# darrenjkt/SEE-VCN

Hardware: AMD Instinct MI355X
Metric: scenes/sec (VCN+voxel+spconv fwd+bwd) (higher is better)
Workload: dtype f32; 1 GPU; VCN_VC fwd on 64 objects x 1024 pts -> kNN surface select (k=30) -> largest DBSCAN cluster (eps 0.4) -> unique + replace (<0.1 m) into 16 KITTI-shaped 64-beam scenes (21.0k pts in range each) -> DynMeanVFE -> VoxelBackBone8x + HeightCompression fwd+bwd + SGD (BASELINE configs[1]+[2]); scenes_per_gpu=16, objects_per_gpu=64, points_per_object=1024, geometry=KITTI [0,-40,-3,70.4,40,1] @ [0.05,0.05,0.1] -> sparse [41,1600,1408], parallelism=dp1, input_side=side stream, one batch ahead (every step = 1 front + 1 compute)

## Files before the change

### include/seevcn_hip.h

```cpp
#ifndef SEEVCN_HIP_H
#define SEEVCN_HIP_H

#include <stddef.h>
#include <stdint.h>

#ifdef __cplusplus
extern "C" {
#endif

#define SV_OK 0
#define SV_ERR_ARG 1
#define SV_ERR_HIP 2

#define SV_ABI_VERSION 1

int sv_abi_version(void);
const char* sv_last_error(void);
int sv_measure_build(void);

size_t sv_index_persistent_bytes(int64_t ncells);
size_t sv_index_scratch_bytes(int64_t ncells);

size_t sv_voxelize_dynamic_scratch_bytes(int64_t num_points, int64_t ncells, int64_t capacity);
int sv_voxelize_dynamic(const float* points, int64_t num_points, int point_stride, int num_features,
// ... 32 lines not shown
int sv_gemm_tn(const float* A, int64_t lda, const float* B, int64_t ldb, float* C, int64_t ldc, int64_t M, int N, int K, void* scratch, void* stream);
size_t sv_gemm_strided_scratch_bytes(int rows, int cols, int64_t contraction);
int sv_gemm_strided(const float* A, int64_t stride_a_row, int64_t stride_a_c, const float* B, int64_t stride_b_c, int64_t stride_b_col, float* C, int64_t ldc,
                    int rows, int cols, int64_t contraction, void* scratch, void* stream);
size_t sv_column_sums_scratch_bytes(int64_t M, int N);
int sv_column_sums(const float* A, int64_t lda, int64_t M, int N, float* out, void* scratch, void* stream);
int sv_segment_max(const float* x, int64_t ldx, int groups, int rows_per_group, int channels, float* out, int32_t* arg, void* stream);
int sv_segment_max_backward(const float* dout, const int32_t* arg, int groups, int rows_per_group, int channels, float* dx, int64_t ldx, void* stream);
int sv_segment_sum(const float* x, int64_t ldx, int groups, int rows_per_group, int channels, float* out, void* stream);
int sv_act_backward(const float* dy, const float* y, int64_t n, int act, float slope, float* dz, void* stream);

int sv_vcn_vc_prep(const float* input, int batch, int n, float* fview, float* centred, float* state, void* stream);
int sv_vcn_vc_pose(const float* fview, int batch, int n, const float* rel_pose, float* state, float* pc_cn, void* stream);
int sv_vcn_vc_finish(const float* coarse_cn, int batch, int num_coarse, const float* state, float* coarse,
                     float* reg_rot, float* reg_centre, void* stream);
int sv_vcn_cn_transform(const float* in, int batch, int n, const float* gt_boxes, int inverse, float* out, void* stream);

int sv_conv_out_shape(const int32_t* in_shape_host, const int32_t* ksize_host, const int32_t* stride_host,
                      const int32_t* padding_host, const int32_t* dilation_host, int32_t* out_shape_host);
size_t sv_rulebook_scratch_bytes(int64_t n_in, int64_t ncells);
int sv_rulebook_subm(const int32_t* coords, int64_t n, int batch, const int32_t* shape_host,
                     const int32_t* ksize_host, const int32_t* dilation_host, void* index_ws, void* scratch,
                     int32_t* nbr, void* stream);
size_t sv_cellmap_persistent_bytes(int batch, const int32_t* spatial_shape);
int sv_rulebook_subm_cellmap(const int32_t* coords, int64_t n, int batch, const int32_t* spatial_shape, const int32_t* ksize,
                             const int32_t* dilation, void* cellmap, int32_t* nbr, int32_t* table_rows, int32_t* masks, void* stream);
int sv_rulebook_sparse(const int32_t* coords, int64_t n_in, int batch, const int32_t* in_shape_host,
                       const int32_t* ksize_host, const int32_t* stride_host, const int32_t* padding_host,
                       const int32_t* dilation_host, void* index_ws, void* scratch, int32_t* out_coords,
                       int32_t* nbr_in, int32_t* in_block, int64_t capacity, int32_t* num_out, void* stream);
size_t sv_rulebook_chain_scratch_bytes(int64_t max_ncells);
int sv_rulebook_chain_count(const int32_t* coords0, int64_t n0, const int32_t* n0_dev, int batch, int n_levels, const int32_t* geoms_host,
                            void* const* index_ws, int32_t* const* sites, const int64_t* caps, int32_t* num_out, void* scratch, void* stream);
int sv_rulebook_batch(const int64_t* jobs_host, int n_jobs, void* stream);
int sv_rulebook_invert(const int32_t* nbr_in, int64_t n_in, int K, int32_t* nbr_out, int64_t n_out, void* stream);
int sv_rulebook_invert_rows(const int32_t* table_rows_in, int64_t n_in, int K, int32_t* out_block, int64_t n_out, void* stream);
int sv_rulebook_pair_counts(const int32_t* nbr, int64_t n_out, int K, int32_t* counts, void* stream);

int sv_sparse_conv_gather_gemm(const float* X, int64_t n_src, const int32_t* nbr, const float* Wt, float* Y,
                               int64_t n_rows, int K, int Kd, int Nc, const float* bias, const float* scale, const float* shift,
                               const float* residual, int relu, void* stream);

int sv_conv_table_rows(const int32_t* nbr, int64_t n_rows, int K, int32_t* table_rows, int32_t* masks, void* stream);
size_t sv_conv_plan_persistent_bytes(void);
size_t sv_conv_plan_perm_bytes(int64_t n_rows);
int sv_conv_plan_build(const int32_t* masks, int64_t n_rows, void* persistent, int32_t* perm, int32_t* masks_p, void* stream);
int sv_conv_tiles_per_wave(int64_t n_rows, int Kd, int Nc);
size_t sv_conv_plan_tiles_bytes(int64_t n_rows, int tiles_per_wave);
int sv_conv_plan_tiles(const int32_t* masks_p, int64_t n_rows, int tiles_per_wave, int32_t* tile_of, void* stream);
int sv_conv_plan_build_dealt(const int32_t* masks, int64_t n_rows, int tiles_per_wave, int32_t* perm, int32_t* masks_p, int32_t* tile_of,
                             void* stream);
int sv_conv_plan_build_dealt_batch(const int64_t* jobs_host, int n_jobs, void* stream);
int sv_conv_mfma_kernel_applies(int K, int Kd, int Nc, int64_t n_src);
int sv_conv_weight_fragments(const float* W, int64_t stride_k, int64_t stride_cin, int64_t stride_cout, int K, int Cin, int Cout, float* frag_fwd,
                             float* frag_bwd, void* stream);
int sv_conv_weight_fragments_batch(const void* descs_device, int n_layers, int64_t total_units, void* stream);
int sv_conv_next_input_norm(const float* coef, int relu);
int sv_sparse_conv_gather_gemm_planned(const float* X, int64_t n_src, const int32_t* table_rows, const int32_t* perm, const int32_t* masks_p,
                                       const int32_t* tile_of, int tiles_per_wave,
                                       const float* wfrag, float* Y, int64_t n_rows, int K, int Kd, int Nc, const float* bias,
                                       const float* scale, const float* shift, const float* residual, int relu, int table_k_reversed,
                                       float* bn_partial, void* stream);
int sv_sparse_conv_dgrad_planned_bn(const float* dZ, int64_t n_src, const int32_t* table_rows, const int32_t* perm, const int32_t* masks_p,
                                    const int32_t* tile_of, int tiles_per_wave, const float* wfrag, float* dY, int64_t n_rows, int K, int Kd, int Nc,
                                    int table_k_reversed, const float* bn_x, const float* bn_mean, const float* bn_invstd, const float* bn_gamma,
                                    const float* bn_beta, int bn_relu, float* bn_partial, void* stream);
// ... 456 lines not shown
```

### see-vcn_amd/_lib.py

```python
import ctypes
import os

import torch

_HERE = os.path.dirname(os.path.abspath(__file__))
LIB_PATH = os.environ.get("SEEVCN_LIB") or os.path.join(_HERE, "lib", "libseevcn_hip.so")
HEADER_PATH = os.path.join(os.path.dirname(_HERE), "include", "seevcn_hip.h")

c_p = ctypes.c_void_p
c_i = ctypes.c_int
c_i64 = ctypes.c_int64
c_f = ctypes.c_float
c_d = ctypes.c_double
c_sz = ctypes.c_size_t

SIGNATURES = {
    "sv_abi_version": (c_i, []),
    "sv_last_error": (ctypes.c_char_p, []),
    "sv_measure_build": (c_i, []),
    "sv_index_persistent_bytes": (c_sz, [c_i64]),
    "sv_index_scratch_bytes": (c_sz, [c_i64]),
    "sv_voxelize_dynamic_scratch_bytes": (c_sz, [c_i64, c_i64, c_i64]),
    "sv_voxelize_dynamic": (c_i, [c_p, c_i64, c_i, c_i, c_p, c_p, c_p, c_i, c_p, c_p, c_p, c_p, c_p, c_i64, c_p, c_p]),
    "sv_mean_vfe": (c_i, [c_p, c_p, c_i64, c_i, c_i, c_p, c_p]),
    "sv_fill_f32": (c_i, [c_p, c_i64, c_f, c_p]),
    "sv_mean_square_scratch_bytes": (ctypes.c_size_t, []),
    "sv_mean_square": (c_i, [c_p, c_i64, c_f, c_f, c_p, c_p, c_p, c_p]),
    "sv_scale_by_device_scalar": (c_i, [c_p, c_i64, c_p, c_p]),
    "sv_gemm_bias_act": (c_i, [c_p, c_i, c_p, c_i, c_p, c_p, c_i, c_p, c_i, c_p, c_i, c_i, c_i, c_i, c_f, c_p]),
    "sv_gemm_splitk_splits": (c_i, [c_i, c_i, c_i]),
    "sv_gemm_splitk_scratch_bytes": (c_sz, [c_i, c_i, c_i]),
    "sv_gemm_bias_act_splitk": (c_i, [c_p, c_i, c_p, c_i, c_p, c_p, c_i, c_p, c_i, c_i, c_i, c_i, c_i, c_f, c_p, c_p]),
    "sv_pointwise_conv3": (c_i, [c_p, c_p, c_p, c_p, c_i64, c_i, c_i, c_f, c_p]),
    "sv_pointwise_conv3_gather": (c_i, [c_p, c_p, c_i64, c_p, c_p, c_p, c_p, c_i, c_i, c_f, c_p]),
    "sv_gemm_tn_scratch_bytes": (c_sz, [c_i64, c_i, c_i]),
    "sv_gemm_tn": (c_i, [c_p, c_i64, c_p, c_i64, c_p, c_i64, c_i64, c_i, c_i, c_p, c_p]),
    "sv_gemm_strided_scratch_bytes": (c_sz, [c_i, c_i, c_i64]),
    "sv_gemm_strided": (c_i, [c_p, c_i64, c_i64, c_p, c_i64, c_i64, c_p, c_i64, c_i, c_i, c_i64, c_p, c_p]),
    "sv_column_sums_scratch_bytes": (c_sz, [c_i64, c_i]),
    "sv_column_sums": (c_i, [c_p, c_i64, c_i64, c_i, c_p, c_p, c_p]),
    "sv_segment_max": (c_i, [c_p, c_i64, c_i, c_i, c_i, c_p, c_p, c_p]),
    "sv_segment_max_backward": (c_i, [c_p, c_p, c_i, c_i, c_i, c_p, c_i64, c_p]),
    "sv_segment_sum": (c_i, [c_p, c_i64, c_i, c_i, c_i, c_p, c_p]),
    "sv_act_backward": (c_i, [c_p, c_p, c_i64, c_i, c_f, c_p, c_p]),
    "sv_vcn_vc_prep": (c_i, [c_p, c_i, c_i, c_p, c_p, c_p, c_p]),
    "sv_vcn_vc_pose": (c_i, [c_p, c_i, c_i, c_p, c_p, c_p, c_p]),
    "sv_vcn_vc_finish": (c_i, [c_p, c_i, c_i, c_p, c_p, c_p, c_p, c_p]),
    "sv_vcn_cn_transform": (c_i, [c_p, c_i, c_i, c_p, c_i, c_p, c_p]),
    "sv_conv_out_shape": (c_i, [c_p, c_p, c_p, c_p, c_p, c_p]),
    "sv_rulebook_scratch_bytes": (c_sz, [c_i64, c_i64]),
    "sv_rulebook_subm": (c_i, [c_p, c_i64, c_i, c_p, c_p, c_p, c_p, c_p, c_p, c_p]),
    "sv_cellmap_persistent_bytes": (c_sz, [c_i, c_p]),
    "sv_rulebook_subm_cellmap": (c_i, [c_p, c_i64, c_i, c_p, c_p, c_p, c_p, c_p, c_p, c_p, c_p]),
    "sv_rulebook_sparse": (c_i, [c_p, c_i64, c_i, c_p, c_p, c_p, c_p, c_p, c_p, c_p, c_p, c_p, c_p, c_i64, c_p, c_p]),
    "sv_rulebook_chain_scratch_bytes": (c_sz, [c_i64]),
    "sv_rulebook_chain_count": (c_i, [c_p, c_i64, c_p, c_i, c_i, c_p, c_p, c_p, c_p, c_p, c_p, c_p]),
    "sv_rulebook_batch": (c_i, [c_p, c_i, c_p]),
    "sv_rulebook_invert": (c_i, [c_p, c_i64, c_i, c_p, c_i64, c_p]),
    "sv_rulebook_invert_rows": (c_i, [c_p, c_i64, c_i, c_p, c_i64, c_p]),
    "sv_rulebook_pair_counts": (c_i, [c_p, c_i64, c_i, c_p, c_p]),
    "sv_sparse_conv_gather_gemm": (c_i, [c_p, c_i64, c_p, c_p, c_p, c_i64, c_i, c_i, c_i, c_p, c_p, c_p, c_p, c_i, c_p]),
    "sv_conv_plan_persistent_bytes": (c_sz, []),
    "sv_conv_table_rows": (c_i, [c_p, c_i64, c_i, c_p, c_p, c_p]),
    "sv_conv_plan_perm_bytes": (c_sz, [c_i64]),
    "sv_conv_plan_build": (c_i, [c_p, c_i64, c_p, c_p, c_p, c_p]),
    "sv_sparse_conv_gather_gemm_planned": (c_i, [c_p, c_i64, c_p, c_p, c_p, c_p, c_i, c_p, c_p, c_i64, c_i, c_i, c_i, c_p, c_p, c_p, c_p, c_i, c_i, c_p, c_p]),
    "sv_sparse_conv_dgrad_planned_bn": (c_i, [c_p, c_i64, c_p, c_p, c_p, c_p, c_i, c_p, c_p, c_i64, c_i, c_i, c_i, c_i, c_p, c_p, c_p, c_p, c_p, c_i, c_p, c_p]),
    "sv_conv_planned_partials": (c_i, []),
    "sv_conv_h16_applies": (c_i, [c_i, c_i, c_i, c_i64]),
    "sv_conv_weight_fragments_h16": (c_i, [c_p, c_i64, c_i64, c_i64, c_i, c_i, c_i, c_p, c_p]),
    "sv_conv_weight_fragments_h16_batch": (c_i, [c_p, c_i, c_i64, c_p]),
    "sv_sparse_conv_gather_gemm_planned_h16": (c_i, [c_p, c_i64, c_p, c_p, c_p, c_p, c_p, c_i, c_i64, c_i, c_i, c_i, c_p, c_p, c_p, c_p, c_i, c_p]),
    "sv_narrow_h16": (c_i, [c_p, c_i64, c_p, c_p]),
    "sv_batchnorm_relu_forward_partial": (c_i, [c_p, c_i64, c_i, c_p, c_p, c_p, c_p, c_f, c_f, c_i, c_p, c_i, c_p, c_p, c_p, c_p, c_p]),
    "sv_debug_conv_trace": (c_i, [c_p]),
    "sv_debug_wgrad_trace": (c_i, [c_p]),
    "sv_conv_tiles_per_wave": (c_i, [c_i64, c_i, c_i]),
    "sv_conv_plan_tiles_bytes": (c_sz, [c_i64, c_i]),
    "sv_conv_weight_fragments_batch": (c_i, [c_p, c_i, c_i64, c_p]),
    "sv_conv_plan_build_dealt": (c_i, [c_p, c_i64, c_i, c_p, c_p, c_p, c_p]),
    "sv_conv_plan_tiles": (c_i, [c_p, c_i64, c_i, c_p, c_p]),
    "sv_conv_plan_build_dealt_batch": (c_i, [c_p, c_i, c_p]),
    "sv_conv_mfma_kernel_applies": (c_i, [c_i, c_i, c_i, c_i64]),
    "sv_conv_weight_fragments": (c_i, [c_p, c_i64, c_i64, c_i64, c_i, c_i, c_i, c_p, c_p, c_p]),
    "sv_sparse_conv_wgrad_scratch_bytes": (c_sz, [c_i64, c_i, c_i, c_i]),
    "sv_sparse_conv_wgrad": (c_i, [c_p, c_i64, c_p, c_p, c_p, c_i64, c_i, c_i, c_i, c_p, c_p]),
    "sv_sparse_conv_wgrad_strided": (c_i, [c_p, c_i64, c_p, c_p, c_p, c_i64, c_i, c_i, c_i, c_i64, c_i64, c_i64, c_p, c_p]),
    "sv_sparse_conv_wgrad_partial_bytes": (c_sz, [c_i64, c_i, c_i, c_i]),
    "sv_sparse_conv_wgrad_stage1": (c_i, [c_p, c_i64, c_p, c_p, c_p, c_i64, c_i, c_i, c_i, c_i64, c_i64, c_i64, c_p, c_p, c_p]),
# ... 344 lines not shown
```

### see-vcn_amd/csrc/rulebook.hip

```cpp
#include "common.h"
#include "wave.h"

struct ConvGeom {
  int batch;
  int in_shape[3];
  int out_shape[3];
  int ksize[3];
  int stride[3];
  int pad[3];
  int dil[3];
  int K;
};

constexpr int RB_THREADS = 256;

__device__ __forceinline__ int64_t lin_key(int b, int z, int y, int x, const int* shape) {
  return (((int64_t)b * shape[0] + z) * shape[1] + y) * shape[2] + x;
}

__device__ __forceinline__ bool coord_ok(const int4 c, int batch, const int* shape) {
  return c.x >= 0 && c.x < batch && c.y >= 0 && c.y < shape[0] && c.z >= 0 && c.z < shape[1] && c.w >= 0 && c.w < shape[2];
}

__global__ __launch_bounds__(RB_THREADS) void k_index_prefix(SvIndexView ix, int64_t nchunks) {
  const int lane = threadIdx.x & 63;
  const int64_t wave = ((int64_t)blockIdx.x * blockDim.x + threadIdx.x) >> 6;
  const int64_t nwaves = ((int64_t)gridDim.x * blockDim.x) >> 6;
  for (int64_t c0 = wave * 64; c0 < nchunks; c0 += nwaves * 64) {
    const int64_t c = c0 + lane;
    const int cnt = c < nchunks ? ix.chunk_cnt[c] : 0;
    unsigned long long occ = __ballot(cnt > 0);
    while (occ) {
// ... 549 lines not shown
  }
  if ((threadIdx.x & 63) == 0 && local) atomicAdd(&counts[k], local);
}

extern "C" int sv_rulebook_pair_counts(const int32_t* nbr, int64_t n_out, int K, int32_t* counts, void* stream) {
  SV_CHECK_ARG(K > 0 && n_out >= 0 && counts, "rulebook_pair_counts: bad arguments");
  hipStream_t st = sv_stream(stream);
  SV_HIP(hipMemsetAsync(counts, 0, (size_t)K * 4, st));
  if (n_out == 0) return SV_OK;
  SV_CHECK_ARG(nbr, "rulebook_pair_counts: null pointer");
  dim3 grid(sv_grid_1d(n_out, RB_THREADS, 64), K);
  hipLaunchKernelGGL(k_pair_count, grid, dim3(RB_THREADS), 0, st, nbr, n_out, K, counts);
  SV_LAUNCH_CHECK();
  return SV_OK;
}

constexpr int CH_BLOCK = 256;
constexpr int CH_MAX_LEVELS = 8;
constexpr int CH_EMIT_SPLIT = 4;
static_assert(CH_BLOCK == RB_THREADS, "k_chain_emit scans one chunk count per thread");
static bool small_kernel_host(const ConvGeom& g) { return g.ksize[0] <= 3 && g.ksize[1] <= 3 && g.ksize[2] <= 3; }

template <bool FULL3>
__global__ __launch_bounds__(RB_THREADS) void k_chain_mark_list(const int4* __restrict__ coords, const int32_t* __restrict__ n_dev, int64_t n_host,
                                                                ConvGeom g, SvIndexView ix) {
  int64_t n = n_dev ? (int64_t)*n_dev : n_host;
  if (n > n_host) n = n_host;
  for (int64_t i = (int64_t)blockIdx.x * blockDim.x + threadIdx.x; i < n; i += (int64_t)gridDim.x * blockDim.x) {
    const int4 c = coords[i];
    if (coord_ok(c, g.batch, g.in_shape)) sparse_mark_one<FULL3>(c, g, ix, 0);
  }
}

__global__ __launch_bounds__(RB_THREADS) void k_chain_count(SvIndexView ix, int64_t nchunks, int32_t* __restrict__ block_sums) {
  __shared__ int s_sum[RB_THREADS / 32];
  constexpr int PER = CH_BLOCK / (RB_THREADS / 32);
  const int lane = threadIdx.x & 31, sub = threadIdx.x >> 5;
  const int64_t c0 = (int64_t)blockIdx.x * CH_BLOCK;
  uint32_t bits[PER];
#pragma unroll
  for (int i = 0; i < PER; ++i) {
    const int64_t c = c0 + sub + (RB_THREADS / 32) * i;
    bits[i] = c < nchunks ? ix.words[c * SV_CHUNK_WORDS + lane].x : 0u;
  }
  int mine = 0;
#pragma unroll
  for (int i = 0; i < PER; ++i) {
    const unsigned long long any = __ballot(bits[i] != 0u);
    if (!((any >> (32 * (sub & 1))) & 0xffffffffull)) continue;
    const int64_t c = c0 + sub + (RB_THREADS / 32) * i;
    const int p = __popc(bits[i]);
    const int incl = sv_wave_incl_scan<32>(p);
    if (bits[i]) ix.words[c * SV_CHUNK_WORDS + lane].y = (uint32_t)(incl - p);
    if (lane == 31) ix.chunk_cnt[c] = incl, mine += incl;
  }
  if (lane == 31) s_sum[sub] = mine;
  __syncthreads();
  if (threadIdx.x == 0) {
    int t = 0;
#pragma unroll
    for (int i = 0; i < RB_THREADS / 32; ++i) t += s_sum[i];
    block_sums[blockIdx.x] = t;
  }
}

__global__ __launch_bounds__(RB_THREADS) void k_chain_emit(SvIndexView ix, int64_t nchunks, const int32_t* __restrict__ block_sums, int4* __restrict__ sites,
                                                           int64_t capacity, int32_t* __restrict__ num_out, ConvGeom gout ) {
  __shared__ int s_red[RB_THREADS / SV_WAVE], s_wtot[RB_THREADS / SV_WAVE], s_wne[RB_THREADS / SV_WAVE];
  __shared__ int s_cbase[CH_BLOCK];
  __shared__ uint16_t s_list[CH_BLOCK];
  const int tid = threadIdx.x, lane32 = tid & 31, sub = tid >> 5, b = blockIdx.x, lane = tid & 63, wid = tid >> 6;
  int before = 0;
  for (int j = tid; j < b; j += RB_THREADS) before += block_sums[j];
  before = sv_wave_reduce_sum(before);
  const int64_t c_mine = (int64_t)b * CH_BLOCK + tid;
  const int cnt = c_mine < nchunks ? ix.chunk_cnt[c_mine] : 0;
  const int incl = sv_wave_incl_scan(cnt);
  const unsigned long long ne = __ballot(cnt > 0);
  if (lane == 0) s_red[wid] = before, s_wne[wid] = __popcll(ne);
  if (lane == 63) s_wtot[wid] = incl;
  __syncthreads();
  int base = 0, wbase = 0, total = 0, nebase = 0, n_ne = 0;
#pragma unroll
  for (int i = 0; i < RB_THREADS / SV_WAVE; ++i) {
    base += s_red[i];
    if (i < wid) wbase += s_wtot[i], nebase += s_wne[i];
    total += s_wtot[i], n_ne += s_wne[i];
  }
  s_cbase[tid] = base + wbase + incl - cnt;
  if (cnt > 0) s_list[nebase + __popcll(ne & ((1ull << lane) - 1ull))] = (uint16_t)tid;
  if (b == (int)gridDim.x - 1 && blockIdx.y == 0 && tid == 0) *num_out = base + total;
  __syncthreads();
  const int q_lo = (int)((int64_t)n_ne * blockIdx.y / gridDim.y), q_hi = (int)((int64_t)n_ne * (blockIdx.y + 1) / gridDim.y);
  const int X = gout.out_shape[2], Y = gout.out_shape[1], Z = gout.out_shape[0];
  const bool narrow = ix.ncells < ((int64_t)1 << 31);
  constexpr int EM_B = 4, GROUPS = RB_THREADS / 32;
  for (int q0 = q_lo + sub; q0 < q_hi; q0 += GROUPS * EM_B) {
    uint2 wd[EM_B];
    int jj[EM_B];
#pragma unroll
    for (int u = 0; u < EM_B; ++u) {
      const int q = q0 + GROUPS * u;
      jj[u] = q < q_hi ? (int)s_list[q] : -1;
      wd[u] = jj[u] >= 0 ? ix.words[((int64_t)b * CH_BLOCK + jj[u]) * SV_CHUNK_WORDS + lane32] : make_uint2(0u, 0u);
    }
#pragma unroll
    for (int u = 0; u < EM_B; ++u) {
      uint32_t bits = wd[u].x;
      if (!bits) continue;
      const int64_t w = ((int64_t)b * CH_BLOCK + jj[u]) * SV_CHUNK_WORDS + lane32;
      int64_t r = (int64_t)s_cbase[jj[u]] + wd[u].y;
      int bb, z0, y0, x0;
      if (narrow) {
        const uint32_t key = (uint32_t)w * 32u;
        const uint32_t q1 = key / (uint32_t)X;
        x0 = (int)(key - q1 * (uint32_t)X);
        const uint32_t q2 = q1 / (uint32_t)Y;
        y0 = (int)(q1 - q2 * (uint32_t)Y);
        bb = (int)(q2 / (uint32_t)Z);
        z0 = (int)(q2 - (uint32_t)bb * (uint32_t)Z);
      } else {
        const int64_t key = w * 32;
        const int64_t q1 = key / X, q2 = q1 / Y;
        x0 = (int)(key - q1 * X), y0 = (int)(q1 - q2 * Y), bb = (int)(q2 / Z), z0 = (int)(q2 - (int64_t)bb * Z);
      }
      while (bits) {
        const int bit = __ffs(bits) - 1;
        bits &= bits - 1u;
        int x = x0 + bit, y = y0, z = z0, bq = bb;
        while (x >= X) {
          x -= X;
          if (++y == Y) {
            y = 0;
            if (++z == Z) z = 0, ++bq;
          }
        }
        if (r < capacity) sites[r] = make_int4(bq, z, y, x);
        ++r;
      }
    }
  }
}

extern "C" size_t sv_rulebook_chain_scratch_bytes(int64_t max_ncells) {
  return align256((size_t)(sv_index_nchunks(max_ncells) / CH_BLOCK + 2) * sizeof(int32_t));
}

extern "C" int sv_rulebook_chain_count(const int32_t* coords0, int64_t n0, const int32_t* n0_dev, int batch, int n_levels, const int32_t* geoms_host,
                                       void* const* index_ws, int32_t* const* sites, const int64_t* caps, int32_t* num_out, void* scratch, void* stream) {
  SV_CHECK_ARG(batch > 0 && n_levels >= 1 && n_levels <= CH_MAX_LEVELS && n0 >= 0 && geoms_host && index_ws && sites && caps && num_out && scratch,
               "rulebook_chain_count: bad arguments (1 <= levels <= %d)", CH_MAX_LEVELS);
  SV_CHECK_ARG(coords0 || n0 == 0, "rulebook_chain_count: null coordinates");
  hipStream_t st = sv_stream(stream);
  ConvGeom g[CH_MAX_LEVELS];
  SvIndexView ix[CH_MAX_LEVELS];
  bool full3[CH_MAX_LEVELS];
  for (int l = 0; l < n_levels; ++l) {
    const int32_t* q = geoms_host + 15 * l;
    int rc = fill_geom(g[l], batch, q, q + 3, q + 6, q + 9, q + 12, false);
    if (rc) return rc;
    SV_CHECK_ARG(g[l].K <= RB_KMAX && small_kernel_host(g[l]), "rulebook_chain_count: kernels up to 3 per axis");
    if (l > 0)
      for (int d = 0; d < 3; ++d) SV_CHECK_ARG(g[l].in_shape[d] == g[l - 1].out_shape[d], "rulebook_chain_count: level %d does not take level %d's output shape", l, l - 1);
    SV_CHECK_ARG(index_ws[l] && sites[l] && caps[l] > 0, "rulebook_chain_count: null pointer at level %d", l);
    const int64_t ncells = (int64_t)batch * g[l].out_shape[0] * g[l].out_shape[1] * g[l].out_shape[2];
    ix[l] = sv_index_view(index_ws[l], ncells);
    full3[l] = g[l].ksize[0] == 3 && g[l].ksize[1] == 3 && g[l].ksize[2] == 3;
  }
  const int4* c4 = reinterpret_cast<const int4*>(coords0);
  if (n0 > 0) {
    const dim3 grid(sv_grid_1d(n0, RB_THREADS, 2048));
    if (full3[0]) hipLaunchKernelGGL(k_chain_mark_list<true>, grid, dim3(RB_THREADS), 0, st, c4, n0_dev, n0, g[0], ix[0]);
    else hipLaunchKernelGGL(k_chain_mark_list<false>, grid, dim3(RB_THREADS), 0, st, c4, n0_dev, n0, g[0], ix[0]);
  }
  int32_t* sums = reinterpret_cast<int32_t*>(scratch);
  for (int l = 0; l < n_levels; ++l) {
    const int64_t nchunks = sv_index_nchunks(ix[l].ncells);
    const int blocks = (int)((nchunks + CH_BLOCK - 1) / CH_BLOCK);
    int4* s4 = reinterpret_cast<int4*>(sites[l]);
    hipLaunchKernelGGL(k_chain_count, dim3(blocks), dim3(RB_THREADS), 0, st, ix[l], nchunks, sums);
    hipLaunchKernelGGL(k_chain_emit, dim3(blocks, CH_EMIT_SPLIT), dim3(RB_THREADS), 0, st, ix[l], nchunks, sums, s4, caps[l], num_out + l, g[l]);
    if (l + 1 < n_levels) {
      const dim3 grid(sv_grid_1d(caps[l], RB_THREADS, 2048));
      if (full3[l + 1]) hipLaunchKernelGGL(k_chain_mark_list<true>, grid, dim3(RB_THREADS), 0, st, s4, num_out + l, caps[l], g[l + 1], ix[l + 1]);
      else hipLaunchKernelGGL(k_chain_mark_list<false>, grid, dim3(RB_THREADS), 0, st, s4, num_out + l, caps[l], g[l + 1], ix[l + 1]);
    }
  }
  SV_LAUNCH_CHECK();
  return SV_OK;
}

constexpr int RBJ_MAX = 16;

struct SetJob {
  const int4* src;
  int4* dst;
  int32_t* map;
  uint2* words;
  int32_t* chunk_cnt;
  int64_t n;
  int shape[3];
  int batch;
  CellTiling t;
  int wg0;
};
struct SetBatch { SetJob j[RBJ_MAX]; int n; };

template <typename B>
__device__ __forceinline__ int job_of_block(const B& b, int blk) {
  int j = 0;
#pragma unroll
  for (int q = 1; q < RBJ_MAX; ++q) j += (q < b.n && blk >= b.j[q].wg0) ? 1 : 0;
  return j;
}

__global__ __launch_bounds__(RB_THREADS) void k_batch_set(SetBatch b, int clear_only) {
  const int ji = job_of_block(b, blockIdx.x);
  const SetJob& J = b.j[ji];
  const int64_t i = (int64_t)(blockIdx.x - J.wg0) * RB_THREADS + threadIdx.x;
  if (i >= J.n) return;
// ... 157 lines not shown
```

### see-vcn_amd/spconv/functional.py

```python
import ctypes
import math
import os
import weakref

import torch

from .. import _lib


def _i3(v):
    v = list(v) if isinstance(v, (list, tuple)) else [v, v, v]
    assert len(v) == 3
    return _lib.host_array(ctypes.c_int32, [int(x) for x in v])


def conv_out_shape(in_shape, ksize, stride, padding, dilation):
    lib = _lib.load()
    out = (ctypes.c_int32 * 3)()
    _lib.check(lib.sv_conv_out_shape(_i3(in_shape), _i3(ksize), _i3(stride), _i3(padding), _i3(dilation), out), "sv_conv_out_shape")
    return [int(x) for x in out]


class _ArenaViews:
    _arena = None
# ... 196 lines not shown
    def pair_counts(self):
        lib = _lib.load()
        counts = torch.empty((self.K,), dtype=torch.int32, device=self.nbr_out.device)
        _lib.check(lib.sv_rulebook_pair_counts(_lib.ptr(self.nbr_out), self.n_out, self.K, _lib.ptr(counts), _lib.stream()),
                   "sv_rulebook_pair_counts")
        return counts


class MirrorRulebook(Rulebook):

    def __init__(self, paired):
        assert not paired.subm and paired.nbr_in is not None and paired.in_indices is not None
        super().__init__(paired.nbr_in, paired.nbr_out, paired.in_indices, list(paired.in_shape), paired.n_out, paired.n_in, False, list(paired.ksize))
        self.paired = paired
        self._K = paired.K
        self.rows_out, self.masks_out, self.rows_in, self.masks_in = paired.rows_in, paired.masks_in, paired.rows_out, paired.masks_out
        self.in_indices, self.in_shape = paired.out_indices, list(paired.out_shape)

    def _table_plan(self, key, n_rows, g):
        return self.paired._table_plan("bwd" if key == "fwd" else "fwd", n_rows, g)

    def plan_addrs(self, direction, kd, nc):
        p = self.plan(direction, kd, nc)
        if p is None:
            return None
        tp, tile_of, g, rev = p
        return tp.addr("rows"), tp.addr("perm"), tp.addr("masks_p"), tile_of.data_ptr(), g, rev


CELLMAP_MAX_BYTES = int(os.environ.get("SEEVCN_CELLMAP_MAX_BYTES", 24 << 30))
FUSED_PLAN = os.environ.get("SEEVCN_FUSED_PLAN", "1") != "0"
USE_PLAN = os.environ.get("SEEVCN_SPCONV_PLAN", "1") != "0"
WGRAD_PLANNED = os.environ.get("SEEVCN_WGRAD_PLANNED", "1") != "0"


def build_subm_rulebook(indices, batch_size, spatial_shape, ksize, dilation=(1, 1, 1)):
    lib = _lib.load()
    _lib.require_cuda(indices)
    assert indices.dtype == torch.int32 and indices.dim() == 2 and indices.shape[1] == 4
    indices = indices.contiguous()
    n = indices.shape[0]
    dev = indices.device
    K = int(ksize[0]) * int(ksize[1]) * int(ksize[2])
    ncells = int(batch_size) * int(spatial_shape[0]) * int(spatial_shape[1]) * int(spatial_shape[2])
    nbr = torch.empty((K, n), dtype=torch.int32, device=dev)
    map_bytes = lib.sv_cellmap_persistent_bytes(int(batch_size), _i3(spatial_shape))
    if map_bytes <= CELLMAP_MAX_BYTES:
        cellmap = _lib.workspace.persistent(f"rb_cellmap_{tuple(spatial_shape)}", map_bytes, dev)
        with_rows = K <= 27 and n > 0
        rows = torch.empty((n, 32), dtype=torch.int32, device=dev) if with_rows else None
        masks = torch.empty((n,), dtype=torch.int32, device=dev) if with_rows else None
        rc = lib.sv_rulebook_subm_cellmap(_lib.ptr(indices), n, int(batch_size), _i3(spatial_shape), _i3(ksize), _i3(dilation),
                                          _lib.ptr(cellmap), _lib.ptr(nbr), _lib.ptr(rows), _lib.ptr(masks), _lib.stream())
        _lib.check(rc, "sv_rulebook_subm_cellmap")
        rb = Rulebook(nbr, None, indices, list(spatial_shape), n, n, True, list(ksize))
        rb.rows_out, rb.masks_out = rows, masks
        rb.dilation = [int(d) for d in dilation]
        return rb
    ws = _lib.workspace.persistent(f"rb_index_{tuple(spatial_shape)}_{batch_size}", lib.sv_index_persistent_bytes(ncells), dev)
    scratch = _lib.workspace.scratch("rb_scratch", lib.sv_rulebook_scratch_bytes(n, ncells), dev)
    rc = lib.sv_rulebook_subm(_lib.ptr(indices), n, int(batch_size), _i3(spatial_shape), _i3(ksize), _i3(dilation),
                              _lib.ptr(ws), _lib.ptr(scratch), _lib.ptr(nbr), _lib.stream())
    _lib.check(rc, "sv_rulebook_subm")
    rb = Rulebook(nbr, None, indices, list(spatial_shape), n, n, True, list(ksize))
    rb.dilation = [int(d) for d in dilation]
    return rb
# ... 38 lines not shown
    rb = Rulebook(nbr_out, nbr_in, out_coords, oshape, n_in, n_out, False, list(ksize))
    rb.rows_out, rb.masks_out = out_block[:32 * n_out].view(n_out, 32), out_block[(32 + K) * n_out:]
    rb.rows_in, rb.masks_in = in_block[:32 * n_in].view(n_in, 32), in_block[32 * n_in:]
    return rb


class ConvSpec:
    __slots__ = ("key", "subm", "ksize", "stride", "padding", "dilation", "cin", "cout")

    def __init__(self, key, subm, ksize, stride, padding, dilation, cin, cout):
        self.key, self.subm = key, bool(subm)
        self.ksize, self.stride, self.padding, self.dilation = ([int(v) for v in t] for t in (ksize, stride, padding, dilation))
        self.cin, self.cout = int(cin), int(cout)


def _al(n, q=64):
    return (int(n) + q - 1) // q * q


def build_network_index(coords, batch_size, spatial_shape, specs, n0_dev=None, with_backward=True):
    import numpy as np
    lib = _lib.load()
    _lib.require_cuda(coords)
    assert coords.dtype == torch.int32 and coords.dim() == 2 and coords.shape[1] == 4
    coords = coords.contiguous()
    dev, B, cap0 = coords.device, int(batch_size), int(coords.shape[0])
    strided = [sp for sp in specs if not sp.subm]
    if cap0 == 0 or not specs or len(strided) > 8 or any(max(sp.ksize) > 3 for sp in specs) or any(not (k & 1) for sp in specs if sp.subm for k in sp.ksize):
        return None
    shapes = [[int(v) for v in spatial_shape]]
    for sp in strided:
        shapes.append(conv_out_shape(shapes[-1], sp.ksize, sp.stride, sp.padding, sp.dilation))
    L = len(strided)
    map_bytes = [lib.sv_cellmap_persistent_bytes(B, _i3(sh)) for sh in shapes]
    if max(map_bytes) > CELLMAP_MAX_BYTES:
        return None
    ncells = [B * sh[0] * sh[1] * sh[2] for sh in shapes]
    counts = None
    if L:
        caps, cap = [], cap0
        for l, sp in enumerate(strided):
            per_in = 1
            for k, st, dl in zip(sp.ksize, sp.stride, sp.dilation):
                per_in *= -(-k // st) if math.gcd(dl, st) == 1 else k
            cap = max(min(cap * per_in, ncells[l + 1]), 1)
            caps.append(cap)
        works = [_lib.workspace.persistent(f"rb_index_{tuple(shapes[l + 1])}_{B}", lib.sv_index_persistent_bytes(ncells[l + 1]), dev) for l in range(L)]
        assert len({w.data_ptr() for w in works}) == L, "two levels of a chain on one grid would share their index"
        sites = [_lib.workspace.scratch(f"rb_chain_sites_{l}", caps[l] * 16, dev) for l in range(L)]
        scratch = _lib.workspace.scratch("rb_chain_scratch", lib.sv_rulebook_chain_scratch_bytes(max(ncells[1:])), dev)
        num_out = torch.empty((L,), dtype=torch.int32, device=dev)
        geoms = []
        for l, sp in enumerate(strided):
            geoms += shapes[l] + sp.ksize + sp.stride + sp.padding + sp.dilation
        rc = lib.sv_rulebook_chain_count(_lib.ptr(coords), cap0, _lib.ptr(n0_dev), B, L, _lib.host_array(ctypes.c_int32, geoms),
                                         _lib.host_array(ctypes.c_void_p, [w.data_ptr() for w in works]),
                                         _lib.host_array(ctypes.c_void_p, [t.data_ptr() for t in sites]), _lib.host_array(ctypes.c_int64, caps),
                                         _lib.ptr(num_out), _lib.ptr(scratch), _lib.stream())
        _lib.check(rc, "sv_rulebook_chain_count")
    try:
        if L:
            vals = _lib.host_ints(([n0_dev] if n0_dev is not None else []) + [num_out])
        else:
            vals = _lib.host_ints([n0_dev]) if n0_dev is not None else []
        n = [vals.pop(0) if n0_dev is not None else cap0] + vals
        if any(n[l + 1] > caps[l] for l in range(L)):
            raise _lib.SeevcnHipError(f"build_network_index: a strided level emitted {n[1:]} output sites for capacities {caps}")
    except BaseException:
        if L:
            for w in works:
                w.zero_()
        raise
    if n[0] != cap0:
        coords = coords[:n[0]]
    total = [0]

    def take(count):
        off = total[0]
        total[0] += _al(max(int(count), 0))
        return off, int(count)

    level_of, lv, tables, plans = {}, 0, {}, []
    for sp in specs:
        K = sp.ksize[0] * sp.ksize[1] * sp.ksize[2]
        if sp.subm:
            if sp.key not in tables:
                tables[sp.key] = dict(spec=sp, level=lv, K=K, nbr=take(K * n[lv]), rows=take(32 * n[lv]), masks=take(n[lv]), plans={})
            t = tables[sp.key]
            assert t["spec"].subm and t["spec"].ksize == sp.ksize and t["level"] == lv, f"indice_key {sp.key} reused with a different kernel or level"
        else:
            assert sp.key not in tables, f"indice_key {sp.key} used by two strided convolutions"
            tables[sp.key] = dict(spec=sp, level=lv, K=K, out_idx=take(4 * n[lv + 1]), nbr_in=take(K * n[lv]), in_block=take(33 * n[lv]),
# ... 495 lines not shown
```

Baseline: 4560 scenes/sec.

## Build all strided-level voxel indices directly from input coords in three launches

Adds a direct chain path that marks output occupancy for every strided level in a single pass over the input coordinates. It tracks per-axis reachable coordinate sets, at most three per axis, through the level chain, so levels are not computed one after another from each other's output sites. Count and emit then run as single batched launches covering all levels, which replaces a per-level sequence of kernels and their dependencies. The cost is more atomic ORs per input point and a host-side geometry check (cached) to confirm the axis-set bound holds; otherwise it falls back to the old chain.

```diff
diff --git a/include/seevcn_hip.h b/include/seevcn_hip.h
--- a/include/seevcn_hip.h
+++ b/include/seevcn_hip.h
@@ -88,6 +88,10 @@
 size_t sv_rulebook_chain_scratch_bytes(int64_t max_ncells);
 int sv_rulebook_chain_count(const int32_t* coords0, int64_t n0, const int32_t* n0_dev, int batch, int n_levels, const int32_t* geoms_host,
                             void* const* index_ws, int32_t* const* sites, const int64_t* caps, int32_t* num_out, void* scratch, void* stream);
+int sv_rulebook_chain_direct_applies(int n_levels, const int32_t* geoms_host);
+size_t sv_rulebook_chain_direct_scratch_bytes(int n_levels, const int64_t* ncells_host);
+int sv_rulebook_chain_direct(const int32_t* coords0, int64_t n0, const int32_t* n0_dev, int batch, int n_levels, const int32_t* geoms_host,
+                             void* const* index_ws, int32_t* const* sites, const int64_t* caps, int32_t* num_out, void* scratch, void* stream);
 int sv_rulebook_batch(const int64_t* jobs_host, int n_jobs, void* stream);
 int sv_rulebook_invert(const int32_t* nbr_in, int64_t n_in, int K, int32_t* nbr_out, int64_t n_out, void* stream);
 int sv_rulebook_invert_rows(const int32_t* table_rows_in, int64_t n_in, int K, int32_t* out_block, int64_t n_out, void* stream);
diff --git a/see-vcn_amd/_lib.py b/see-vcn_amd/_lib.py
--- a/see-vcn_amd/_lib.py
+++ b/see-vcn_amd/_lib.py
@@ -55,6 +55,9 @@
     "sv_rulebook_sparse": (c_i, [c_p, c_i64, c_i, c_p, c_p, c_p, c_p, c_p, c_p, c_p, c_p, c_p, c_p, c_i64, c_p, c_p]),
     "sv_rulebook_chain_scratch_bytes": (c_sz, [c_i64]),
     "sv_rulebook_chain_count": (c_i, [c_p, c_i64, c_p, c_i, c_i, c_p, c_p, c_p, c_p, c_p, c_p, c_p]),
+    "sv_rulebook_chain_direct_applies": (c_i, [c_i, c_p]),
+    "sv_rulebook_chain_direct_scratch_bytes": (c_sz, [c_i, c_p]),
+    "sv_rulebook_chain_direct": (c_i, [c_p, c_i64, c_p, c_i, c_i, c_p, c_p, c_p, c_p, c_p, c_p, c_p]),
     "sv_rulebook_batch": (c_i, [c_p, c_i, c_p]),
     "sv_rulebook_invert": (c_i, [c_p, c_i64, c_i, c_p, c_i64, c_p]),
     "sv_rulebook_invert_rows": (c_i, [c_p, c_i64, c_i, c_p, c_i64, c_p]),
diff --git a/see-vcn_amd/csrc/rulebook.hip b/see-vcn_amd/csrc/rulebook.hip
--- a/see-vcn_amd/csrc/rulebook.hip
+++ b/see-vcn_amd/csrc/rulebook.hip
@@ -1,3 +1,5 @@
+#include <string.h>
+
 #include "common.h"
 #include "wave.h"
 
@@ -613,11 +615,11 @@
   }
 }
 
-__global__ __launch_bounds__(RB_THREADS) void k_chain_count(SvIndexView ix, int64_t nchunks, int32_t* __restrict__ block_sums) {
+__device__ __forceinline__ void chain_count_block(const SvIndexView& ix, int64_t nchunks, int32_t* __restrict__ block_sums, int blk) {
   __shared__ int s_sum[RB_THREADS / 32];
   constexpr int PER = CH_BLOCK / (RB_THREADS / 32);
   const int lane = threadIdx.x & 31, sub = threadIdx.x >> 5;
-  const int64_t c0 = (int64_t)blockIdx.x * CH_BLOCK;
+  const int64_t c0 = (int64_t)blk * CH_BLOCK;
   uint32_t bits[PER];
 #pragma unroll
   for (int i = 0; i < PER; ++i) {
@@ -641,16 +643,21 @@
     int t = 0;
 #pragma unroll
     for (int i = 0; i < RB_THREADS / 32; ++i) t += s_sum[i];
-    block_sums[blockIdx.x] = t;
-  }
-}
-
-__global__ __launch_bounds__(RB_THREADS) void k_chain_emit(SvIndexView ix, int64_t nchunks, const int32_t* __restrict__ block_sums, int4* __restrict__ sites,
-                                                           int64_t capacity, int32_t* __restrict__ num_out, ConvGeom gout ) {
+    block_sums[blk] = t;
+  }
+}
+
+__global__ __launch_bounds__(RB_THREADS) void k_chain_count(SvIndexView ix, int64_t nchunks, int32_t* __restrict__ block_sums) {
+  chain_count_block(ix, nchunks, block_sums, blockIdx.x);
+}
+
+__device__ __forceinline__ void chain_emit_block(const SvIndexView& ix, int64_t nchunks, const int32_t* __restrict__ block_sums, int4* __restrict__ sites,
+                                                 int64_t capacity, int32_t* __restrict__ num_out, const int* shape, int b, int nblocks, int share,
+                                                 int nshares) {
   __shared__ int s_red[RB_THREADS / SV_WAVE], s_wtot[RB_THREADS / SV_WAVE], s_wne[RB_THREADS / SV_WAVE];
   __shared__ int s_cbase[CH_BLOCK];
   __shared__ uint16_t s_list[CH_BLOCK];
-  const int tid = threadIdx.x, lane32 = tid & 31, sub = tid >> 5, b = blockIdx.x, lane = tid & 63, wid = tid >> 6;
+  const int tid = threadIdx.x, lane32 = tid & 31, sub = tid >> 5, lane = tid & 63, wid = tid >> 6;
   int before = 0;
   for (int j = tid; j < b; j += RB_THREADS) before += block_sums[j];
   before = sv_wave_reduce_sum(before);
@@ -670,10 +677,10 @@
   }
   s_cbase[tid] = base + wbase + incl - cnt;
   if (cnt > 0) s_list[nebase + __popcll(ne & ((1ull << lane) - 1ull))] = (uint16_t)tid;
-  if (b == (int)gridDim.x - 1 && blockIdx.y == 0 && tid == 0) *num_out = base + total;
+  if (b == nblocks - 1 && share == 0 && tid == 0) *num_out = base + total;
   __syncthreads();
-  const int q_lo = (int)((int64_t)n_ne * blockIdx.y / gridDim.y), q_hi = (int)((int64_t)n_ne * (blockIdx.y + 1) / gridDim.y);
-  const int X = gout.out_shape[2], Y = gout.out_shape[1], Z = gout.out_shape[0];
+  const int q_lo = (int)((int64_t)n_ne * share / nshares), q_hi = (int)((int64_t)n_ne * (share + 1) / nshares);
+  const int X = shape[2], Y = shape[1], Z = shape[0];
   const bool narrow = ix.ncells < ((int64_t)1 << 31);
   constexpr int EM_B = 4, GROUPS = RB_THREADS / 32;
   for (int q0 = q_lo + sub; q0 < q_hi; q0 += GROUPS * EM_B) {
@@ -721,6 +728,11 @@
       }
     }
   }
+}
+
+__global__ __launch_bounds__(RB_THREADS) void k_chain_emit(SvIndexView ix, int64_t nchunks, const int32_t* __restrict__ block_sums, int4* __restrict__ sites,
+                                                           int64_t capacity, int32_t* __restrict__ num_out, ConvGeom gout ) {
+  chain_emit_block(ix, nchunks, block_sums, sites, capacity, num_out, gout.out_shape, blockIdx.x, gridDim.x, blockIdx.y, gridDim.y);
 }
 
 extern "C" size_t sv_rulebook_chain_scratch_bytes(int64_t max_ncells) {
@@ -767,6 +779,207 @@
       else hipLaunchKernelGGL(k_chain_mark_list<false>, grid, dim3(RB_THREADS), 0, st, s4, num_out + l, caps[l], g[l + 1], ix[l + 1]);
     }
   }
+  SV_LAUNCH_CHECK();
+  return SV_OK;
+}
+
+constexpr int CH_AXIS_SET = 3;
+
+struct ChainMarkAll {
+  ConvGeom g[CH_MAX_LEVELS];
+  uint2* words[CH_MAX_LEVELS];
+  int n;
+};
+struct ChainLevel {
+  SvIndexView ix;
+  int64_t nchunks;
+  int4* sites;
+  int64_t cap;
+  int32_t* sums;
+  int shape[3];
+  int wg0, nblocks;
+};
+struct ChainLevels { ChainLevel lv[CH_MAX_LEVELS]; int n; };
+static_assert(sizeof(ChainMarkAll) <= 3900 && sizeof(ChainLevels) <= 3900, "kernel argument block");
+
+__device__ __forceinline__ int level_of_block(const ChainLevels& b, int blk) {
+  int l = 0;
+#pragma unroll
+  for (int q = 1; q < CH_MAX_LEVELS; ++q) l += (q < b.n && blk >= b.lv[q].wg0) ? 1 : 0;
+  return l;
+}
+
+__device__ __forceinline__ void axis_set_insert(int (&a)[CH_AXIS_SET], int o) {
+  if (o < 0 || o == a[0] || o == a[1] || o == a[2]) return;
+  if (a[0] < 0) a[0] = o;
+  else if (a[1] < 0) a[1] = o;
+  else if (a[2] < 0) a[2] = o;
+}
+static_assert(CH_AXIS_SET == 3, "axis_set_insert and k_chain_mark_all name the three slots");
+
+__global__ __launch_bounds__(RB_THREADS) void k_chain_mark_all(const int4* __restrict__ coords, const int32_t* __restrict__ n_dev, int64_t n_host,
+                                                               ChainMarkAll m) {
+  int64_t n = n_dev ? (int64_t)*n_dev : n_host;
+  if (n > n_host) n = n_host;
+  const int lane = threadIdx.x & (SV_WAVE - 1);
+  for (int64_t i = (int64_t)blockIdx.x * blockDim.x + threadIdx.x; i - lane < n; i += (int64_t)gridDim.x * blockDim.x) {
+    const int4 c = i < n ? coords[i] : make_int4(-1, -1, -1, -1);
+    const bool ok = coord_ok(c, m.g[0].batch, m.g[0].in_shape);
+    int a[3][CH_AXIS_SET] = {{ok ? c.y : -1, -1, -1}, {ok ? c.z : -1, -1, -1}, {ok ? c.w : -1, -1, -1}};
+    const bool below = lane > 0 && ok && __shfl_up(c.x, 1) == c.x;
+    for (int l = 0; l < m.n; ++l) {
+      const ConvGeom& g = m.g[l];
+      bool dup[3][CH_AXIS_SET];
+#pragma unroll
+      for (int ax = 0; ax < 3; ++ax) {
+        const int s = g.stride[ax];
+        int nx[CH_AXIS_SET] = {-1, -1, -1};
+#pragma unroll
+        for (int q = 0; q < CH_AXIS_SET; ++q) {
+#pragma unroll
+          for (int ka = 0; ka < 3; ++ka) {
+            int o = -1;
+            if (a[ax][q] >= 0 && ka < g.ksize[ax]) {
+              const int t = a[ax][q] + g.pad[ax] - ka * g.dil[ax];
+              if (t >= 0) {
+                if (s == 1) o = t;
+                else if (s == 2) o = (t & 1) ? -1 : (t >> 1);
+                else o = (t % s) ? -1 : t / s;
+                if (o >= g.out_shape[ax]) o = -1;
+              }
+            }
+            axis_set_insert(nx, o);
+          }
+        }
+        const int b0 = __shfl_up(nx[0], 1), b1 = __shfl_up(nx[1], 1), b2 = __shfl_up(nx[2], 1);
+#pragma unroll
+        for (int q = 0; q < CH_AXIS_SET; ++q) {
+          a[ax][q] = nx[q];
+          dup[ax][q] = nx[q] == b0 || nx[q] == b1 || nx[q] == b2;
+        }
+      }
+      uint2* const words = m.words[l];
+#pragma unroll
+      for (int qz = 0; qz < CH_AXIS_SET; ++qz)
+#pragma unroll
+        for (int qy = 0; qy < CH_AXIS_SET; ++qy)
+#pragma unroll
+          for (int qx = 0; qx < CH_AXIS_SET; ++qx) {
+            const int z = a[0][qz], y = a[1][qy], x = a[2][qx];
+            if ((z | y | x) < 0) continue;
+            if (below && dup[0][qz] && dup[1][qy] && dup[2][qx]) continue;
+            const int64_t key = lin_key(c.x, z, y, x, g.out_shape);
+            __hip_atomic_fetch_or(&words[key >> 5].x, 1u << (key & 31), __ATOMIC_RELAXED, __HIP_MEMORY_SCOPE_AGENT);
+          }
+    }
+  }
+}
+
+__global__ __launch_bounds__(RB_THREADS) void k_chain_count_all(ChainLevels b) {
+  const int l = level_of_block(b, blockIdx.x);
+  const ChainLevel& J = b.lv[l];
+  chain_count_block(J.ix, J.nchunks, J.sums, blockIdx.x - J.wg0);
+}
+
+__global__ __launch_bounds__(RB_THREADS) void k_chain_emit_all(ChainLevels b, int32_t* __restrict__ num_out) {
+  const int l = level_of_block(b, blockIdx.x);
+  const ChainLevel& J = b.lv[l];
+  chain_emit_block(J.ix, J.nchunks, J.sums, J.sites, J.cap, num_out + l, J.shape, blockIdx.x - J.wg0, J.nblocks, blockIdx.y, gridDim.y);
+}
+
+static int chain_geoms(ConvGeom* g, int batch, int n_levels, const int32_t* geoms_host, const char* who) {
+  for (int l = 0; l < n_levels; ++l) {
+    const int32_t* q = geoms_host + 15 * l;
+    int rc = fill_geom(g[l], batch, q, q + 3, q + 6, q + 9, q + 12, false);
+    if (rc) return rc;
+    SV_CHECK_ARG(g[l].K <= RB_KMAX && small_kernel_host(g[l]), "%s: kernels up to 3 per axis", who);
+    if (l > 0)
+      for (int d = 0; d < 3; ++d) SV_CHECK_ARG(g[l].in_shape[d] == g[l - 1].out_shape[d], "%s: level %d does not take level %d's output shape", who, l, l - 1);
+  }
+  return SV_OK;
+}
+
+static int chain_direct_walk(int n_levels, const int32_t* geoms_host);
+extern "C" int sv_rulebook_chain_direct_applies(int n_levels, const int32_t* geoms_host) {
+  if (n_levels < 1 || n_levels > CH_MAX_LEVELS || !geoms_host) return 0;
+  thread_local int32_t last[15 * CH_MAX_LEVELS];
+  thread_local int last_levels = 0, last_answer = 0;
+  if (last_levels == n_levels && !memcmp(last, geoms_host, sizeof(int32_t) * 15 * n_levels)) return last_answer;
+  last_answer = chain_direct_walk(n_levels, geoms_host);
+  memcpy(last, geoms_host, sizeof(int32_t) * 15 * n_levels);
+  last_levels = n_levels;
+  return last_answer;
+}
+static int chain_direct_walk(int n_levels, const int32_t* geoms_host) {
+  ConvGeom g[CH_MAX_LEVELS];
+  for (int l = 0; l < n_levels; ++l) {
+    const int32_t* q = geoms_host + 15 * l;
+    if (fill_geom(g[l], 1, q, q + 3, q + 6, q + 9, q + 12, false) || g[l].K > RB_KMAX || !small_kernel_host(g[l])) return 0;
+    if (l > 0)
+      for (int d = 0; d < 3; ++d)
+        if (g[l].in_shape[d] != g[l - 1].out_shape[d]) return 0;
+  }
+  for (int ax = 0; ax < 3; ++ax)
+    for (int v0 = 0; v0 < g[0].in_shape[ax]; ++v0) {
+      int set[3 * CH_AXIS_SET], ns = 1;
+      set[0] = v0;
+      for (int l = 0; l < n_levels && ns > 0; ++l) {
+        int nx[3 * CH_AXIS_SET], nn = 0;
+        for (int q = 0; q < ns; ++q)
+          for (int ka = 0; ka < g[l].ksize[ax]; ++ka) {
+            const int t = set[q] + g[l].pad[ax] - ka * g[l].dil[ax];
+            if (t < 0 || t % g[l].stride[ax] || t / g[l].stride[ax] >= g[l].out_shape[ax]) continue;
+            const int o = t / g[l].stride[ax];
+            bool seen = false;
+            for (int r = 0; r < nn; ++r) seen |= nx[r] == o;
+            if (!seen) nx[nn++] = o;
+          }
+        if (nn > CH_AXIS_SET) return 0;
+        for (int r = 0; r < nn; ++r) set[r] = nx[r];
+        ns = nn;
+      }
+    }
+  return 1;
+}
+
+extern "C" size_t sv_rulebook_chain_direct_scratch_bytes(int n_levels, const int64_t* ncells_host) {
+  size_t ints = 0;
+  for (int l = 0; l < n_levels && l < CH_MAX_LEVELS && ncells_host; ++l) ints += (size_t)(sv_index_nchunks(ncells_host[l]) / CH_BLOCK + 2);
+  return align256(ints * sizeof(int32_t));
+}
+
+extern "C" int sv_rulebook_chain_direct(const int32_t* coords0, int64_t n0, const int32_t* n0_dev, int batch, int n_levels, const int32_t* geoms_host,
+                                        void* const* index_ws, int32_t* const* sites, const int64_t* caps, int32_t* num_out, void* scratch, void* stream) {
+  SV_CHECK_ARG(batch > 0 && n_levels >= 1 && n_levels <= CH_MAX_LEVELS && n0 >= 0 && geoms_host && index_ws && sites && caps && num_out && scratch,
+               "rulebook_chain_direct: bad arguments (1 <= levels <= %d)", CH_MAX_LEVELS);
+  SV_CHECK_ARG(coords0 || n0 == 0, "rulebook_chain_direct: null coordinates");
+  SV_CHECK_ARG(sv_rulebook_chain_direct_applies(n_levels, geoms_host), "rulebook_chain_direct: an input reaches more than %d coordinates per axis at some level "
+               "(or bad geometry): use sv_rulebook_chain_count", CH_AXIS_SET);
+  hipStream_t st = sv_stream(stream);
+  ChainMarkAll m;
+  ChainLevels lv;
+  int rc = chain_geoms(m.g, batch, n_levels, geoms_host, "rulebook_chain_direct");
+  if (rc) return rc;
+  m.n = lv.n = n_levels;
+  int32_t* sums = reinterpret_cast<int32_t*>(scratch);
+  int wgs = 0;
+  for (int l = 0; l < n_levels; ++l) {
+    SV_CHECK_ARG(index_ws[l] && sites[l] && caps[l] > 0, "rulebook_chain_direct: null pointer at level %d", l);
+    ChainLevel& J = lv.lv[l];
+    J.ix = sv_index_view(index_ws[l], (int64_t)batch * m.g[l].out_shape[0] * m.g[l].out_shape[1] * m.g[l].out_shape[2]);
+    m.words[l] = J.ix.words;
+    J.nchunks = sv_index_nchunks(J.ix.ncells);
+    J.sites = reinterpret_cast<int4*>(sites[l]), J.cap = caps[l], J.sums = sums;
+    for (int d = 0; d < 3; ++d) J.shape[d] = m.g[l].out_shape[d];
+    J.nblocks = (int)((J.nchunks + CH_BLOCK - 1) / CH_BLOCK);
+    J.wg0 = wgs;
+    wgs += J.nblocks;
+    sums += J.nblocks + 1;
+  }
+  if (n0 > 0)
+    hipLaunchKernelGGL(k_chain_mark_all, dim3(sv_grid_1d(n0, RB_THREADS, 2048)), dim3(RB_THREADS), 0, st, reinterpret_cast<const int4*>(coords0), n0_dev, n0, m);
+  hipLaunchKernelGGL(k_chain_count_all, dim3(wgs), dim3(RB_THREADS), 0, st, lv);
+  hipLaunchKernelGGL(k_chain_emit_all, dim3(wgs, CH_EMIT_SPLIT), dim3(RB_THREADS), 0, st, lv, num_out);
   SV_LAUNCH_CHECK();
   return SV_OK;
 }
diff --git a/see-vcn_amd/spconv/functional.py b/see-vcn_amd/spconv/functional.py
--- a/see-vcn_amd/spconv/functional.py
+++ b/see-vcn_amd/spconv/functional.py
@@ -252,6 +252,7 @@
 FUSED_PLAN = os.environ.get("SEEVCN_FUSED_PLAN", "1") != "0"
 USE_PLAN = os.environ.get("SEEVCN_SPCONV_PLAN", "1") != "0"
 WGRAD_PLANNED = os.environ.get("SEEVCN_WGRAD_PLANNED", "1") != "0"
+INDEX_DIRECT = os.environ.get("SEEVCN_INDEX_DIRECT", "1") != "0"
 
 
 def build_subm_rulebook(indices, batch_size, spatial_shape, ksize, dilation=(1, 1, 1)):
@@ -356,6 +357,8 @@
     for sp in strided:
         shapes.append(conv_out_shape(shapes[-1], sp.ksize, sp.stride, sp.padding, sp.dilation))
     L = len(strided)
+    if len({tuple(sh) for sh in shapes}) <= L:
+        return None
     map_bytes = [lib.sv_cellmap_persistent_bytes(B, _i3(sh)) for sh in shapes]
     if max(map_bytes) > CELLMAP_MAX_BYTES:
         return None
@@ -372,16 +375,23 @@
         works = [_lib.workspace.persistent(f"rb_index_{tuple(shapes[l + 1])}_{B}", lib.sv_index_persistent_bytes(ncells[l + 1]), dev) for l in range(L)]
         assert len({w.data_ptr() for w in works}) == L, "two levels of a chain on one grid would share their index"
         sites = [_lib.workspace.scratch(f"rb_chain_sites_{l}", caps[l] * 16, dev) for l in range(L)]
-        scratch = _lib.workspace.scratch("rb_chain_scratch", lib.sv_rulebook_chain_scratch_bytes(max(ncells[1:])), dev)
         num_out = torch.empty((L,), dtype=torch.int32, device=dev)
         geoms = []
         for l, sp in enumerate(strided):
             geoms += shapes[l] + sp.ksize + sp.stride + sp.padding + sp.dilation
-        rc = lib.sv_rulebook_chain_count(_lib.ptr(coords), cap0, _lib.ptr(n0_dev), B, L, _lib.host_array(ctypes.c_int32, geoms),
-                                         _lib.host_array(ctypes.c_void_p, [w.data_ptr() for w in works]),
-                                         _lib.host_array(ctypes.c_void_p, [t.data_ptr() for t in sites]), _lib.host_array(ctypes.c_int64, caps),
-                                         _lib.ptr(num_out), _lib.ptr(scratch), _lib.stream())
-        _lib.check(rc, "sv_rulebook_chain_count")
+        geoms = _lib.host_array(ctypes.c_int32, geoms)
+        direct = INDEX_DIRECT and bool(lib.sv_rulebook_chain_direct_applies(L, geoms))
+        if direct:
+            chain, name = lib.sv_rulebook_chain_direct, "sv_rulebook_chain_direct"
+            scratch_bytes = lib.sv_rulebook_chain_direct_scratch_bytes(L, _lib.host_array(ctypes.c_int64, ncells[1:]))
+        else:
+            chain, name = lib.sv_rulebook_chain_count, "sv_rulebook_chain_count"
+            scratch_bytes = lib.sv_rulebook_chain_scratch_bytes(max(ncells[1:]))
+        scratch = _lib.workspace.scratch("rb_chain_scratch", scratch_bytes, dev)
+        rc = chain(_lib.ptr(coords), cap0, _lib.ptr(n0_dev), B, L, geoms, _lib.host_array(ctypes.c_void_p, [w.data_ptr() for w in works]),
+                   _lib.host_array(ctypes.c_void_p, [t.data_ptr() for t in sites]), _lib.host_array(ctypes.c_int64, caps),
+                   _lib.ptr(num_out), _lib.ptr(scratch), _lib.stream())
+        _lib.check(rc, name)
     try:
         if L:
             vals = _lib.host_ints(([n0_dev] if n0_dev is not None else []) + [num_out])
```

Measured after the change: 4550 scenes/sec. About the same (-0.2%).
